# damaggu/StableKeypoints

Hardware: AMD Instinct MI355X
Metric: images/sec (token-opt step, 512², N=500 tokens) (higher is better)
Workload: dtype f32

## Files before the change

### stablekeypoints_amd/csrc/skp_conv.hip

```cpp
#include <cstdlib>

#include "skp_common.h"
#include "skp_gn.h"

using namespace skp;

#ifndef SKP_WINO_DEBUG
#define SKP_WINO_DEBUG 0
#endif
#ifndef SKP_WINO2_DEBUG
#define SKP_WINO2_DEBUG 0
#endif

namespace {

typedef float f32x4 __attribute__((ext_vector_type(4)));
typedef unsigned int u32x4 __attribute__((ext_vector_type(4)));

constexpr int kMT = 64;
constexpr int kNC = 32;
constexpr int kCK = 4;
constexpr int kP = 36;
constexpr int kThreads = 512;
constexpr int kUs = kCK * kNC * kP;
// ... 334 lines not shown
  SKP_CHECK_ARG(B > 0 && C > 0 && K > 0 && H > 0 && W > 0, "non-positive shape");
  SKP_CHECK_ARG(C % kCK == 0, "input channels must be a multiple of 4");
  SKP_CHECK_ARG(K % kNC == 0, "output channels must be a multiple of 32");
  SKP_CHECK_ARG(H % 4 == 0 && W % 4 == 0, "H and W must be multiples of 4");
  SKP_CHECK_ARG(nsplit >= 1 && C % (kCK * nsplit) == 0, "nsplit must divide C into multiples of 4");
  SKP_CHECK_ARG(nsplit == 1 || ws, "split-K needs a workspace of nsplit·B·K·H·W floats");
  SKP_CHECK_ARG(aligned16(x) && aligned16(U) && aligned16(y) && (!residual || aligned16(residual)) &&
                    (!ws || aligned16(ws)),
                "tensors must be 16-byte aligned");
  const int tw = W / 4, tpi = (H / 4) * tw;
  const long long ntiles = (long long)B * tpi;
  SKP_CHECK_ARG(ntiles <= 0x7fffffffLL - kMT, "too many tiles");
  SKP_CHECK_ARG((long long)B * C * H * W * 4 < 0x7fffffffLL, "input larger than 2 GiB (32-bit buffer offsets)");
  const bool wide = ntiles <= 32 && K % 64 == 0;
  const int mt = wide ? 32 : kMT;
  const int ntb = (int)((ntiles + mt - 1) / mt), nkb = K / (wide ? 64 : kNC);
  SKP_CHECK_ARG((long long)ntb * nkb * nsplit <= 0x7fffffffLL, "grid too large");
  const long long ubytes = (long long)K * C * kP * 4;
  const int kb_major = ubytes > (2LL << 20);
  const int epi = nsplit > 1 ? 0 : (bias ? 1 : 0) | (residual ? 2 : 0);
  float* out = nsplit > 1 ? ws : y;
  const int dbg = SKP_WINO_DEBUG;
  hipStream_t st = as_stream(stream);
  const dim3 grid((unsigned)(ntb * nkb * nsplit));
#define SKP_WG(E)                                                                                                    \
  if (wide)                                                                                                          \
    hipLaunchKernelGGL((wino_f4_kernel<E, 32>), grid, dim3(kThreads), 0, st, x, U, bias, residual, out, B, C, K, H, W, \
                       tw, tpi, (int)ntiles, ntb, nkb, kb_major, C / nsplit, dbg);                                    \
  else                                                                                                               \
    hipLaunchKernelGGL((wino_f4_kernel<E, 64>), grid, dim3(kThreads), 0, st, x, U, bias, residual, out, B, C, K, H, W, \
                       tw, tpi, (int)ntiles, ntb, nkb, kb_major, C / nsplit, dbg)
  switch (epi) {
    case 0: SKP_WG(0); break;
    case 1: SKP_WG(1); break;
    case 2: SKP_WG(2); break;
    default: SKP_WG(3); break;
  }
#undef SKP_WG
  SKP_LAUNCH_CHECK();
  if (nsplit > 1) return splitk_reduce(ws, nsplit, B, K, H * W, bias, residual, y, st);
  return SKP_OK;
}

namespace {
namespace w2 {

constexpr int kNC = 32;
constexpr int kCK = 4;
template <int TXB>
struct Geo;
template <>
struct Geo<8> {
  static constexpr int NI = 1, RR = 34, RC = 10, CHF = 1408;
};
template <>
struct Geo<4> {
  static constexpr int NI = 4, RR = 18, RC = 6, CHF = 1744;
};
template <int TXB, int NW>
struct GeoN : Geo<TXB> {};
template <>
struct GeoN<8, 4> {
  static constexpr int NI = 1, RR = 18, RC = 10, CHF = 768;
};
template <>
struct GeoN<4, 4> {
  static constexpr int NI = 2, RR = 18, RC = 6, CHF = 880;
};
template <int TXB, int NW = 8>
struct GeoT : GeoN<TXB, NW> {
  using GeoN<TXB, NW>::NI;
  using GeoN<TXB, NW>::RR;
  using GeoN<TXB, NW>::RC;
  using GeoN<TXB, NW>::CHF;
  static constexpr int RF = 4 * RC;
  static constexpr int RAWF = (4 * CHF + 255) / 256 * 256;
  static constexpr int RAW_INSTR = RAWF / 256;
  static_assert(NI * RR * RF <= CHF, "channel region");
};
constexpr int kUP = 40;
constexpr int kUF = kCK * kNC * kUP;
constexpr int kUInstr = kUF / 256;
constexpr unsigned kOOB = 0x80000000u;
static_assert(kUF % 256 == 0, "whole 1-KB chunks");
static_assert((4 * GeoT<8>::RAWF + 3 * kUF) * 4 <= 160 * 1024 && 3 * (GeoT<4>::RAWF + kUF) * 4 <= 160 * 1024, "LDS");
static_assert(2 * 8 * 1024 <= kUF * 4, "epilogue exchange: two waves' 8 KB per ring buffer");

__device__ constexpr float kBt[6][6] = {{1.f, -1.5f, -2.f, 1.5f, 1.f, 0.f},  {0.f, -1.f, 0.5f, 2.5f, 1.f, 0.f},
                                        {0.f, 1.f, -2.5f, 0.5f, 1.f, 0.f},  {0.f, -2.f, -1.f, 2.f, 1.f, 0.f},
                                        {0.f, 0.5f, -1.f, -0.5f, 1.f, 0.f}, {0.f, 1.f, -1.5f, -2.f, 1.5f, 1.f}};
__device__ constexpr float kAt[4][6] = {{1.f, 1.f, 1.f, 1.f, 1.f, 0.f},
                                        {0.f, 1.f, -1.f, 0.5f, -2.f, 0.f},
                                        {0.f, 1.f, 1.f, 0.25f, 4.f, 0.f},
                                        {0.f, 1.f, -1.f, 0.125f, -8.f, 1.f}};

#ifndef SKP_W2_PACKED
#define SKP_W2_PACKED 1
#endif
#if SKP_W2_PACKED
#define W2_TRANSFORM half_transform_pk
#else
#define W2_TRANSFORM half_transform
#endif

#define W2_VMCNT(n) __builtin_amdgcn_s_waitcnt(((n) & 15) | (((n) >> 4) << 14) | (7 << 4) | (15 << 8))

template <int H, int RF>
__device__ __forceinline__ void half_transform(const float* raw, float* a) {
  float t[3][6];
#pragma unroll
  for (int r = 0; r < 6; ++r) {
    const float4 c0 = *reinterpret_cast<const float4*>(raw + r * RF);
    const float4 c1 = *reinterpret_cast<const float4*>(raw + r * RF + 4);
    const float4 c2 = *reinterpret_cast<const float4*>(raw + r * RF + 8);
    const float d[6] = {c0.w, c1.x, c1.y, c1.z, c1.w, c2.x};
#pragma unroll
    for (int ii = 0; ii < 3; ++ii) {
      const float c = kBt[3 * H + ii][r];
      if (c == 0.0f) continue;
      bool first = true;
#pragma unroll
      for (int rp = 0; rp < r; ++rp)
        if (kBt[3 * H + ii][rp] != 0.0f) first = false;
#pragma unroll
      for (int b = 0; b < 6; ++b)
        t[ii][b] = first ? ((c == 1.0f) ? d[b] : c * d[b]) : ((c == 1.0f) ? t[ii][b] + d[b] : fmaf(c, d[b], t[ii][b]));
    }
    asm volatile("" ::"v"(c0.x), "v"(c0.y), "v"(c0.z), "v"(c2.y), "v"(c2.z), "v"(c2.w));
  }
#pragma unroll
  for (int ii = 0; ii < 3; ++ii) bt6(t[ii][0], t[ii][1], t[ii][2], t[ii][3], t[ii][4], t[ii][5], a + 6 * ii, 1);
}

typedef float f2 __attribute__((ext_vector_type(2)));

template <typename T>
__device__ __forceinline__ void bt6_shared(T a0, T a1, T a2, T a3, T a4, T a5, T* y) {
  const T e = a4 - a2, f = a3 - a1, g = a2 + a3, h = a3 - a2;
  y[0] = __builtin_elementwise_fma((T)1.5f, f, (a0 + e) - a2);
  y[1] = __builtin_elementwise_fma((T)1.5f, g, e + f);
  y[2] = __builtin_elementwise_fma((T)1.5f, h, e - f);
  y[3] = __builtin_elementwise_fma((T)2.0f, f, e);
  y[4] = __builtin_elementwise_fma((T)-0.5f, f, e);
  y[5] = __builtin_elementwise_fma((T)1.5f, e, __builtin_elementwise_fma((T)-2.0f, f, a5 - a1));
}

template <int H, int RF>
__device__ __forceinline__ void half_transform_pk(const float* raw, float* a) {
  f2 t[3][3];
  f2 k0[3], k1[3], k2[3], k3[3];
#pragma unroll
  for (int r = 0; r < 6; ++r) {
    if (H == 1 && r == 0) continue;
    const f32x4 c0 = *reinterpret_cast<const f32x4*>(raw + r * RF);
    const f32x4 c1 = *reinterpret_cast<const f32x4*>(raw + r * RF + 4);
    const f32x4 c2 = *reinterpret_cast<const f32x4*>(raw + r * RF + 8);
    const f2 d[3] = {__builtin_shufflevector(c1, c1, 0, 1), __builtin_shufflevector(c1, c1, 2, 3),
                     __builtin_shufflevector(c0, c2, 3, 4)};
#pragma unroll
    for (int p = 0; p < 3; ++p) {
      if (H == 0) {
        if (r == 0) k0[p] = d[p];
        if (r == 1) { k1[p] = d[p]; k0[p] = __builtin_elementwise_fma((f2)-1.5f, d[p], k0[p]); }
        if (r == 2) { k2[p] = d[p]; k3[p] = __builtin_elementwise_fma((f2)1.5f, d[p], -k1[p]); }
        if (r == 3) { k1[p] = __builtin_elementwise_fma((f2)1.5f, d[p], -k2[p]); k3[p] = k3[p] + d[p]; }
        if (r == 4) {
// ... 112 lines not shown

  unsigned voff[kMaxRaw];
  int nraw = 0;
#pragma unroll
  for (int m = 0; m < kMaxRaw; ++m) {
    const int gi = wv + NW * m;
    voff[m] = w2::kOOB;
    if (gi < kRawInstr) {
      ++nraw;
      const int f = 64 * gi + lane;
      const int ch = f / (kChF / 4);
      const int e = f - ch * (kChF / 4);
      const int ii = e / (RR * RC), rem = e - ii * (RR * RC);
      const int row = rem / RC, c4 = rem - row * RC;
      const int yy = y0 - 1 + row, xx = x0 - 4 + 4 * c4;
      if (ch < w2::kCK && ii < NI && yy >= 0 && yy < H && xx >= 0 && xx < W)
        voff[m] = (unsigned)((ximg + ((size_t)ii * C + ch) * plane + (size_t)yy * W + xx) * 4);
    }
  }
  const int nuw = (kInstr - 1 - wv) / NW + 1 - nraw;
  const int ufirst = wv + NW * nraw - kRawInstr;
  const int allow_step = RS == 2 ? 0 : US == 2 ? nraw : RS == 4 ? nuw + 2 * nraw : nuw + nraw;
  const int allow_pro = RS == 2 ? nuw + nraw : US == 2 ? nuw + 2 * nraw : RS == 4 ? 2 * nuw + 3 * nraw : 2 * nuw + 2 * nraw;
  const size_t xend = (size_t)(img + NI) * C * plane;
  const float* Ub = U + ((size_t)kb * C + c0) * w2::kNC * kUP;
  const int nst = csplit / w2::kCK;

  auto issue_raw = [&](int t, float* rs_lds) {
    const bool ok = t < nst;
    const size_t off = ((size_t)c0 + (size_t)(ok ? t : 0) * w2::kCK) * plane;
    const __amdgpu_buffer_rsrc_t rx = __builtin_amdgcn_make_buffer_rsrc(
        (void*)(x + off), (short)0, ok ? (int)((xend - off) * 4) : 0, 0x00020000);
#pragma unroll
    for (int m = 0; m < kMaxRaw; ++m)
      if (m < nraw && !(dbg & 4))
        __builtin_amdgcn_raw_ptr_buffer_load_lds(rx, (lds_ptr_t)(rs_lds + 256 * (wv + NW * m)), 16, voff[m], 0, 0, 0);
  };
  auto issue_u = [&](int t, float* us_lds) {
    const __amdgpu_buffer_rsrc_t ru =
        __builtin_amdgcn_make_buffer_rsrc((void*)(Ub + (size_t)t * kUF), (short)0, kUF * 4, 0x00020000);
#pragma unroll
    for (int m = 0; m < kMaxU; ++m)
      if (m < nuw && !(dbg & 8)) {
        const int q = ufirst + NW * m;
        __builtin_amdgcn_raw_ptr_buffer_load_lds(ru, (lds_ptr_t)(us_lds + 256 * q), 16, lane * 16, q * 1024, 0, 0);
      }
  };

  const int kc = lane >> 4;
  const int tx = lane & (TXB - 1);
  const int ty = TXB == 8 ? 2 * wm + ((lane >> 3) & 1) : (lane >> 2) & 3;
  const int roff = kc * kChF + (TXB == 8 ? 0 : wm * RR * kRowF) + 4 * ty * kRowF + 4 * tx;
  const int uoff = (kc * w2::kNC + (lane & 15)) * kUP + 20 * HH;

  f32x4 acc[2][18];
#pragma unroll
  for (int b = 0; b < 2; ++b)
#pragma unroll
    for (int q = 0; q < 18; ++q) acc[b][q] = f32x4{0.f, 0.f, 0.f, 0.f};
  float a0[18], a1[18];

  auto mfmas = [&](const float* us, const float (&acur)[18]) {
#pragma unroll
    for (int b = 0; b < 2; ++b) {
      const float* ub = us + uoff + b * 16 * kUP;
      float u[18];
#pragma unroll
      for (int j = 0; j < 4; ++j) {
        const float4 v = *reinterpret_cast<const float4*>(ub + 4 * j);
        u[4 * j] = v.x;
        u[4 * j + 1] = v.y;
        u[4 * j + 2] = v.z;
        u[4 * j + 3] = v.w;
      }
      const float2 v2 = *reinterpret_cast<const float2*>(ub + 16);
      u[16] = v2.x;
      u[17] = v2.y;
#pragma unroll
      for (int q = 0; q < 18; ++q) acc[b][q] = __builtin_amdgcn_mfma_f32_16x16x4f32(acur[q], u[q], acc[b][q], 0, 0, 0);
    }
  };

  if constexpr (VST) {
    const int bw = W >> 5;
    const size_t tb = (size_t)img * ((H >> 4) * bw) + (size_t)(y0 >> 4) * bw + (x0 >> 5);
    const float* Vb = x + (tb * (size_t)(C / w2::kCK) + (size_t)(c0 / w2::kCK)) * kUF;
    auto issue_vu = [&](int t, float* vs_lds, float* us_lds) {
      const __amdgpu_buffer_rsrc_t rv =
          __builtin_amdgcn_make_buffer_rsrc((void*)(Vb + (size_t)t * kUF), (short)0, kUF * 4, 0x00020000);
      const __amdgpu_buffer_rsrc_t ru =
          __builtin_amdgcn_make_buffer_rsrc((void*)(Ub + (size_t)t * kUF), (short)0, kUF * 4, 0x00020000);
#pragma unroll
      for (int m = 0; m < w2::kUInstr / NW; ++m) {
        const int q = wv + NW * m;
        __builtin_amdgcn_raw_ptr_buffer_load_lds(rv, (lds_ptr_t)(vs_lds + 256 * q), 16, lane * 16, q * 1024, 0, 0);
      }
#pragma unroll
      for (int m = 0; m < w2::kUInstr / NW; ++m) {
        const int q = wv + NW * m;
        __builtin_amdgcn_raw_ptr_buffer_load_lds(ru, (lds_ptr_t)(us_lds + 256 * q), 16, lane * 16, q * 1024, 0, 0);
      }
    };
    static_assert(w2::kUInstr % NW == 0, "whole chunks per wave");
    const int aoff = (kc * 32 + 16 * wm + (lane & 15)) * kUP + 20 * HH;
    auto vstep = [&](int s, const float* Vs, const float* Us, float* Vi, float* Ui) {
      W2_VMCNT(0);
      __syncthreads();
      if (s + 1 < nst) issue_vu(s + 1, Vi, Ui);
      float a[18];
      const float* vb = Vs + aoff;
#pragma unroll
      for (int j = 0; j < 4; ++j) {
        const float4 v = *reinterpret_cast<const float4*>(vb + 4 * j);
        a[4 * j] = v.x;
        a[4 * j + 1] = v.y;
        a[4 * j + 2] = v.z;
        a[4 * j + 3] = v.w;
      }
      const float2 v2 = *reinterpret_cast<const float2*>(vb + 16);
      a[16] = v2.x;
      a[17] = v2.y;
      mfmas(Us, a);
    };
    issue_vu(0, R0, U0);
    for (int s0 = 0; s0 < nst; s0 += 2) {
      vstep(s0, R0, U0, R1, U1);
      if (s0 + 1 < nst) vstep(s0 + 1, R1, U1, R0, U0);
    }
  } else {
    issue_raw(0, R0);
    if (RS == 4) issue_raw(1, R1);
    issue_u(0, U0);
    if (RS >= 3) issue_raw(RS - 2, RS == 4 ? R2 : R1);
    if (US == 3 && nst > 1) issue_u(1, U1);
    issue_raw(RS - 1, RS == 4 ? sm.R3 : RS == 3 ? R2 : R1);
    w2_vmcnt(nst > 1 ? allow_pro : 0);
    __syncthreads();
    w2::W2_TRANSFORM<HH, kRowF>(R0 + roff, a0);

    auto step = [&](int s, float* Rn, float* Us, float* Ri, float* Ui, const float (&acur)[18], float (&anext)[18]) {
      w2_vmcnt(s + 1 < nst ? allow_step : 0);
      __syncthreads();
      if (s + US - 1 < nst) issue_u(s + US - 1, Ui);
      issue_raw(s + RS, Ri);
      const bool tr = s + 1 < nst && !(dbg & 1);
      if (HH == 0) {
        if (tr) w2::W2_TRANSFORM<HH, kRowF>(Rn + roff, anext);
        if (!(dbg & 2)) mfmas(Us, acur);
      } else {
        if (!(dbg & 2)) mfmas(Us, acur);
        if (tr) w2::W2_TRANSFORM<HH, kRowF>(Rn + roff, anext);
      }
    };
    constexpr int PER = RS == 4 ? 12 : RS == 2 ? 2 : 6;
    float* const Rsl[4] = {R0, R1, R2, sm.R3};
    float* const Usl[3] = {U0, U1, U2};
    for (int s0 = 0; s0 < ((dbg & 16) ? 0 : nst); s0 += PER) {
      step(s0, Rsl[1 % RS], Usl[0], Rsl[0], Usl[US - 1], a0, a1);
  #pragma unroll
      for (int j = 1; j < PER; ++j) {
        if (s0 + j < nst) {
          if ((j & 1) == 0) step(s0 + j, Rsl[(j + 1) % RS], Usl[j % US], Rsl[j % RS], Usl[(j + US - 1) % US], a0, a1);
          else step(s0 + j, Rsl[(j + 1) % RS], Usl[j % US], Rsl[j % RS], Usl[(j + US - 1) % US], a1, a0);
        }
      }
    }

  }

  W2_VMCNT(0);
  __syncthreads();
  if (dbg & 32) return;
  constexpr int PH = (TXB == 8 && NW == 4) ? 16 : 32;
  constexpr int PLS = (TXB == 8 ? PH * 32 : NI * 256) + 4;
  float* const P2 = RS == 2 ? U1 : R2;
  auto plane_of = [&](int c) -> float* {
    float* b = (c >> 2) == 0 ? R0 : (c >> 2) == 1 ? R1 : (c >> 2) == 2 ? P2 : U0;
    return b + (c & 3) * PLS + (c >> 2) * 16;
  };
  float* pl = plane_of(lane & 15);
  const int pbase = TXB == 8 ? (4 * (2 * wm + (lane >> 5))) * 32 + 4 * (4 * ((lane >> 4) & 1))
                             : wm * 256 + (4 * (lane >> 4)) * 16;
  constexpr int PW = TXB == 8 ? 32 : 16;
#pragma unroll
  for (int blk = 0; blk < 2; ++blk) {
    if (HH != blk) {
#pragma unroll
      for (int r = 0; r < 4; ++r) {
        float m[18], o[16];
#pragma unroll
        for (int q = 0; q < 18; ++q) m[q] = acc[blk][q][r];
        w2::half_output<HH>(m, o);
#pragma unroll
        for (int f = 0; f < 4; ++f)
          *reinterpret_cast<float4*>(pl + pbase + f * PW + 4 * r) =
              make_float4(o[4 * f], o[4 * f + 1], o[4 * f + 2], o[4 * f + 3]);
      }
    }
    __syncthreads();
    if (HH == blk) {
#pragma unroll
      for (int r = 0; r < 4; ++r) {
        float m[18], o[16];
#pragma unroll
        for (int q = 0; q < 18; ++q) m[q] = acc[blk][q][r];
        w2::half_output<HH>(m, o);
#pragma unroll
        for (int f = 0; f < 4; ++f) {
          float4* d = reinterpret_cast<float4*>(pl + pbase + f * PW + 4 * r);
          const float4 p = *d;
// ... 90 lines not shown
        const float p = r == 0 ? piv[0] : r == 1 ? piv[1] : r == 2 ? piv[2] : piv[3];
        constexpr float inv_n = 1.0f / 512.0f;
        gnp[((size_t)img * K + k) * (size_t)((H >> 4) * (W >> 5)) + seg] =
            make_float2(p + x * inv_n, fmaxf(x2 - x * (x * inv_n), 0.0f));
      }
    }
    if (blk == 0) __syncthreads();
  }
}

template <int EPI, int TXB, int NW = 8>
__global__ __launch_bounds__(NW * WAVE) __attribute__((amdgpu_waves_per_eu(2, 2))) void wino2_kernel(
    const float* __restrict__ x, const float* __restrict__ U, const float* __restrict__ bias,
    const float* __restrict__ res, float* __restrict__ y, int nimg, int C, int K, int H, int W, int bw, int bpi,
    int nblk, int nkb, int kb_major, int csplit, int dbg, float2* __restrict__ gnp) {
  __shared__ __attribute__((aligned(16))) float R0[w2::GeoT<TXB, NW>::RAWF], R1[w2::GeoT<TXB, NW>::RAWF],
      R2[(TXB == 4 && NW == 4) ? 4 : w2::GeoT<TXB, NW>::RAWF],
      R3[(TXB == 8 && NW == 8 && SKP_W2_RS4) ? w2::GeoT<TXB, NW>::RAWF : 4];
  __shared__ __attribute__((aligned(16))) float U0[w2::kUF], U1[w2::kUF], U2[NW == 4 ? 4 : w2::kUF];
  const int G = gridDim.x;
  const int g = blockIdx.x;
  const int Lg = (G % 8 == 0) ? (g % 8) * (G / 8) + g / 8 : g;
  const int sp = Lg / (nblk * nkb);
  const int L = Lg - sp * (nblk * nkb);
  y += (size_t)sp * nimg * K * ((EPI & 4) ? (H / 2) * (W / 2) : H * W);
  int tb, kb;
  if (kb_major) {
    kb = L / nblk;
    tb = L - kb * nblk;
  } else {
    tb = L / nkb;
    kb = L - tb * nkb;
  }
  int img, x0 = 0, y0 = 0;
  if (TXB == 8) {
    img = tb / bpi;
    const int br = tb - img * bpi;
    const int by = br / bw;
    x0 = 32 * (br - by * bw);
    y0 = (NW == 4 ? 16 : 32) * by;
  } else {
    img = (NW == 4 ? 2 : 4) * tb;
  }
  const int wv = __builtin_amdgcn_readfirstlane(threadIdx.x >> 6);
  const W2Smem sm{R0, R1, R2, R3, U0, U1, U2};
  const int c0 = sp * csplit;
  if (wv < NW / 2)
    wino2_body<EPI, 0, TXB, NW>(sm, x, U, bias, res, y, C, K, H, W, img, x0, y0, kb, c0, csplit, wv, dbg, gnp);
  else wino2_body<EPI, 1, TXB, NW>(sm, x, U, bias, res, y, C, K, H, W, img, x0, y0, kb, c0, csplit, wv, dbg, gnp);
}

__global__ void wino2_weights_kernel(const float* __restrict__ w, int K, int C, int flip, float* __restrict__ U) {
  const long long i = blockIdx.x * (long long)blockDim.x + threadIdx.x;
  if (i >= (long long)K * C) return;
  const int k = (int)(i / C), c = (int)(i - (long long)k * C);
  double g[9];
  for (int u = 0; u < 3; ++u)
    for (int v = 0; v < 3; ++v)
      g[3 * u + v] = flip ? (double)w[((size_t)c * K + k) * 9 + (2 - u) * 3 + (2 - v)]
                          : (double)w[((size_t)k * C + c) * 9 + u * 3 + v];
  const double Gm[6][3] = {{1.0, 0.0, 0.0},
                           {1.0 / 3, 1.0 / 3, 1.0 / 3},
                           {-1.0 / 3, 1.0 / 3, -1.0 / 3},
                           {-16.0 / 15, -8.0 / 15, -4.0 / 15},
                           {1.0 / 15, -2.0 / 15, 4.0 / 15},
                           {0.0, 0.0, 1.0}};
  double t[6][3];
  for (int a = 0; a < 6; ++a)
    for (int v = 0; v < 3; ++v) t[a][v] = Gm[a][0] * g[v] + Gm[a][1] * g[3 + v] + Gm[a][2] * g[6 + v];
  float* out = U + (((size_t)(k / w2::kNC) * C + c) * w2::kNC + (k % w2::kNC)) * w2::kUP;
  for (int p = 0; p < w2::kUP; ++p) out[p] = 0.0f;
  for (int a = 0; a < 6; ++a)
    for (int b = 0; b < 6; ++b) {
      const int p = 6 * a + b;
      out[p < 18 ? p : p + 2] = (float)(t[a][0] * Gm[b][0] + t[a][1] * Gm[b][1] + t[a][2] * Gm[b][2]);
    }
}

template <int EPI>
__global__ __launch_bounds__(4 * WAVE) __attribute__((amdgpu_waves_per_eu(2, 2))) void wino2v_kernel(
    const float* __restrict__ V, const float* __restrict__ U, const float* __restrict__ bias,
    const float* __restrict__ res, float* __restrict__ y, int nimg, int C, int K, int H, int W, int bw, int bpi,
    int nblk, int nkb, int kb_major, int csplit, int dbg, float2* __restrict__ gnp) {
  __shared__ __attribute__((aligned(16))) float V0[w2::kUF], V1[w2::kUF], U0[w2::kUF], U1[w2::kUF];
  static_assert(4 * w2::kUF * 4 <= 80 * 1024, "two workgroups per CU");
  const int G = gridDim.x;
  const int g = blockIdx.x;
  const int Lg = (G % 8 == 0) ? (g % 8) * (G / 8) + g / 8 : g;
  const int sp = Lg / (nblk * nkb);
  const int L = Lg - sp * (nblk * nkb);
  y += (size_t)sp * nimg * K * H * W;
  int tb, kb;
  if (kb_major) {
    kb = L / nblk;
    tb = L - kb * nblk;
  } else {
    tb = L / nkb;
    kb = L - tb * nkb;
  }
  const int img = tb / bpi;
  const int br = tb - img * bpi;
  const int by = br / bw;
  const int x0 = 32 * (br - by * bw), y0 = 16 * by;
  const int wv = __builtin_amdgcn_readfirstlane(threadIdx.x >> 6);
  const W2Smem sm{V0, V1, nullptr, nullptr, U0, U1, nullptr};
  const int c0 = sp * csplit;
  if (wv < 2)
    wino2_body<EPI, 0, 8, 4, true>(sm, V, U, bias, res, y, C, K, H, W, img, x0, y0, kb, c0, csplit, wv, dbg, gnp);
  else wino2_body<EPI, 1, 8, 4, true>(sm, V, U, bias, res, y, C, K, H, W, img, x0, y0, kb, c0, csplit, wv, dbg, gnp);
}

template <int GN>
__global__ __launch_bounds__(4 * WAVE) void wino2_vtransform_kernel(
    const float* __restrict__ x, const float* __restrict__ stats, const float* __restrict__ gamma,
    const float* __restrict__ beta, const float* __restrict__ shift, int G, float* __restrict__ V, int C, int H, int W,
    int bw, int bpi) {
  using Geo = w2::GeoT<8, 4>;
  constexpr int RR = Geo::RR, RC = Geo::RC, kChF = Geo::CHF, kRowF = Geo::RF;
  __shared__ __attribute__((aligned(16))) float R[Geo::RAWF];
  __shared__ __attribute__((aligned(16))) float O[w2::kUF];
  const int tid = threadIdx.x, lane = tid & 63;
  const int nst = C / w2::kCK;
  const int tb = blockIdx.x / nst, st = blockIdx.x - tb * nst;
  const int img = tb / bpi;
  const int br = tb - img * bpi;
  const int by = br / bw;
  const int x0 = 32 * (br - by * bw), y0 = 16 * by;
  const int cpg = C / (G > 0 ? G : 1);
  for (int f = tid; f < w2::kCK * RR * RC; f += 4 * WAVE) {
    const int ch = f / (RR * RC), e = f - ch * (RR * RC);
    const int row = e / RC, c4 = e - row * RC;
    const int yy = y0 - 1 + row, xx = x0 - 4 + 4 * c4;
    float4 v = make_float4(0.f, 0.f, 0.f, 0.f);
    if (yy >= 0 && yy < H && xx >= 0 && xx < W) {
      const int c = w2::kCK * st + ch;
      v = *reinterpret_cast<const float4*>(x + (((size_t)img * C + c) * H + yy) * W + xx);
      if (GN) {
        const int grp = img * G + c / cpg;
        const GNCoef k = gn_coef(gamma[c], beta[c], stats[2 * grp], stats[2 * grp + 1]);
        const float t = shift ? shift[(size_t)img * C + c] : 0.0f;
        v.x = gn_elem<GN == 2>(v.x, t, k); v.y = gn_elem<GN == 2>(v.y, t, k);
        v.z = gn_elem<GN == 2>(v.z, t, k); v.w = gn_elem<GN == 2>(v.w, t, k);
      }
    }
    *reinterpret_cast<float4*>(R + ch * kChF + row * kRowF + 4 * c4) = v;
  }
  __syncthreads();
  const int wv = __builtin_amdgcn_readfirstlane(tid >> 6);
  const int HH = wv >> 1, wm = wv & 1;
  const int kc = lane >> 4, tx = lane & 7, ty = 2 * wm + ((lane >> 3) & 1);
  const int roff = kc * kChF + 4 * ty * kRowF + 4 * tx;
  float a[20];
  if (HH == 0) w2::W2_TRANSFORM<0, kRowF>(R + roff, a);
  else w2::W2_TRANSFORM<1, kRowF>(R + roff, a);
  a[18] = a[19] = 0.0f;
  float* o = O + (kc * 32 + 16 * wm + (lane & 15)) * w2::kUP + 20 * HH;
#pragma unroll
  for (int j = 0; j < 5; ++j)
    *reinterpret_cast<float4*>(o + 4 * j) = make_float4(a[4 * j], a[4 * j + 1], a[4 * j + 2], a[4 * j + 3]);
  __syncthreads();
  float4* out = reinterpret_cast<float4*>(V + (size_t)blockIdx.x * w2::kUF);
#pragma unroll
  for (int i = 0; i < w2::kUF / 4 / (4 * WAVE); ++i)
    out[i * 4 * WAVE + tid] = reinterpret_cast<const float4*>(O)[i * 4 * WAVE + tid];
}

}

extern "C" int skp_wino2_weights(const float* w, int K, int C, int flip, float* U, void* stream) {
  SKP_CHECK_ARG(w && U, "null pointer");
  SKP_CHECK_ARG(K > 0 && C > 0, "non-positive shape");
  SKP_CHECK_ARG(K % w2::kNC == 0, "output channels must be a multiple of 32");
  const long long n = (long long)K * C;
  hipLaunchKernelGGL(wino2_weights_kernel, dim3((unsigned)((n + 255) / 256)), dim3(256), 0, as_stream(stream), w, K, C,
                     flip, U);
  SKP_LAUNCH_CHECK();
  return SKP_OK;
}

namespace {
int wino_nt_flag(long long out_bytes, int nsplit) {
  if (nsplit > 1) return 0;
  return out_bytes >= (256LL << 20) ? 128 : 0;
}
}

extern "C" int skp_conv3x3s2_wino2(const float* x, const float* U, const float* bias, float* y, int B, int C, int K,
                                   int H, int W, int nsplit, float* ws, void* stream) {
  SKP_CHECK_ARG(x && U && y, "null pointer");
  SKP_CHECK_ARG(B > 0 && C > 0 && K > 0 && H > 0 && W > 0, "non-positive shape");
  SKP_CHECK_ARG(C % w2::kCK == 0, "input channels must be a multiple of 4");
  SKP_CHECK_ARG(K % w2::kNC == 0, "output channels must be a multiple of 32");
  SKP_CHECK_ARG(H % 32 == 0 && W % 32 == 0, "H and W must be multiples of 32");
  SKP_CHECK_ARG(nsplit >= 1 && C % (w2::kCK * nsplit) == 0, "nsplit must divide C into multiples of 4");
  SKP_CHECK_ARG(nsplit == 1 || ws, "split-K needs a workspace of nsplit·B·K·(H/2)·(W/2) floats");
  SKP_CHECK_ARG(aligned16(x) && aligned16(U) && aligned16(y) && (!ws || aligned16(ws)), "tensors must be 16-byte aligned");
  SKP_CHECK_ARG((long long)B * C * H * W * 4 < 0x7fffffffLL, "input larger than 2 GiB (32-bit buffer offsets)");
  const int bw = W / 32, bpi = (H / 16) * bw;
  const long long nblk = (long long)B * bpi;
  const int nkb = K / w2::kNC;
  SKP_CHECK_ARG(nblk * nkb * nsplit <= 0x7fffffffLL, "grid too large");
  float* out = nsplit > 1 ? ws : y;
  hipStream_t st = as_stream(stream);
  const dim3 grid((unsigned)(nblk * nkb * nsplit));
  const int fl = SKP_WINO2_DEBUG | wino_nt_flag((long long)B * K * (H / 2) * (W / 2) * 4, nsplit);
  if (nsplit == 1 && bias)
    hipLaunchKernelGGL((wino2_kernel<5, 8, 4>), grid, dim3(4 * WAVE), 0, st, x, U, bias, nullptr, out, B, C, K, H, W,
                       bw, bpi, (int)nblk, nkb, 0, C / nsplit, fl, nullptr);
  else
    hipLaunchKernelGGL((wino2_kernel<4, 8, 4>), grid, dim3(4 * WAVE), 0, st, x, U, nullptr, nullptr, out, B, C, K, H,
                       W, bw, bpi, (int)nblk, nkb, 0, C / nsplit, fl, nullptr);
  SKP_LAUNCH_CHECK();
  if (nsplit > 1) return splitk_reduce(ws, nsplit, B, K, (H / 2) * (W / 2), bias, nullptr, y, st);
  return SKP_OK;
}

extern "C" int skp_conv3x3_wino2_gn(const float* x, const float* U, const float* bias, const float* residual, float* y,
                                    int B, int C, int K, int H, int W, int nsplit, float* ws, float* gn_part,
                                    void* stream) {
  SKP_CHECK_ARG(x && U && y, "null pointer");
  SKP_CHECK_ARG(!gn_part || (nsplit == 1 && H % 32 == 0 && W % 32 == 0 && (reinterpret_cast<uintptr_t>(gn_part) & 7) == 0),
                "gn_part: one split, H and W multiples of 32, 8-byte aligned");
  SKP_CHECK_ARG(B > 0 && C > 0 && K > 0 && H > 0 && W > 0, "non-positive shape");
  SKP_CHECK_ARG(C % w2::kCK == 0, "input channels must be a multiple of 4");
  SKP_CHECK_ARG(K % w2::kNC == 0, "output channels must be a multiple of 32");
  const bool g16 = H == 16 && W == 16;
  SKP_CHECK_ARG((H % 32 == 0 && W % 32 == 0) || (g16 && B % 4 == 0),
                "H and W must be multiples of 32, or 16×16 with B a multiple of 4");
  SKP_CHECK_ARG(nsplit >= 1 && C % (w2::kCK * nsplit) == 0, "nsplit must divide C into multiples of 4");
  SKP_CHECK_ARG(nsplit == 1 || ws, "split-K needs a workspace of nsplit·B·K·H·W floats");
  SKP_CHECK_ARG(aligned16(x) && aligned16(U) && aligned16(y) && (!residual || aligned16(residual)) &&
                    (!ws || aligned16(ws)),
                "tensors must be 16-byte aligned");
  SKP_CHECK_ARG((long long)B * C * H * W * 4 < 0x7fffffffLL, "input larger than 2 GiB (32-bit buffer offsets)");
  const int bw = W / 32, bpi = (H / 16) * bw;
  const long long nblk = g16 ? B / 2 : (long long)B * bpi;
  const int nkb = K / w2::kNC;
  SKP_CHECK_ARG(nblk * nkb * nsplit <= 0x7fffffffLL, "grid too large");
  const int dbg = SKP_WINO2_DEBUG;
  const int kb_major = 0;
  const int epi = nsplit > 1 ? 0 : (bias ? 1 : 0) | (residual ? 2 : 0);
  float* out = nsplit > 1 ? ws : y;
  hipStream_t st = as_stream(stream);
  const dim3 grid((unsigned)(nblk * nkb * nsplit));
  const int fl = dbg | wino_nt_flag((long long)B * K * H * W * 4, nsplit);
  float2* gnp = reinterpret_cast<float2*>(gn_part);
#define SKP_WG2(E)                                                                                            \
// ... 110 lines not shown
```

### stablekeypoints_amd/ops.py

```python
import ctypes
import os

import torch

from . import _lib
from ._lib import call, ptr, stream

F32 = torch.float32

_TIMER = None


def set_kernel_timer(timer):
    global _TIMER
    _TIMER = timer


class _NoTimer:
    def __enter__(self):
        return self

    def __exit__(self, *a):
        return False

# ... 1550 lines not shown
def conv3x3_s2(x, weight, bias=None):
    _lib.require_device(x)
    if not conv3x3_s2_eligible(x, weight):
        raise ValueError(f"conv3x3_s2: unsupported x {tuple(x.shape)} / weight {tuple(weight.shape)}")
    x = _c16(x)
    B, C, H, W = x.shape
    K = weight.shape[0]
    y = torch.empty(B, K, H // 2, W // 2, device=x.device, dtype=F32)
    U = _wino_u(weight, False, True)
    b = None if bias is None else _c(bias.detach())
    bmax = max(1, (2 ** 31 - 1) // (C * H * W * 4))
    for b0 in range(0, B, bmax):
        b1 = min(B, b0 + bmax)
        _, nsplit, _ = _wino_plan(b1 - b0, C, K, H, W)
        ws = torch.empty(nsplit, b1 - b0, K, H // 2, W // 2, device=x.device, dtype=F32) if nsplit > 1 else None
        with _timed("skp_conv3x3s2_wino2", 0):
            call("skp_conv3x3s2_wino2", ptr(x[b0:b1]), ptr(U), ptr(b), ptr(y[b0:b1]), b1 - b0, C, K, H, W, nsplit,
                 ptr(ws), stream(x.device))
    return y


def conv3x3(x, weight, bias=None, residual=None):
    _lib.require_device(x)
    if weight.requires_grad:
        raise ValueError("conv3x3: the weight must be frozen (requires_grad=False)")
    B, C, H, W = x.shape
    K = weight.shape[0]
    if tuple(weight.shape[1:]) != (C, 3, 3):
        raise ValueError(f"conv3x3: weight {tuple(weight.shape)} does not fit input {tuple(x.shape)}")
    if residual is not None and tuple(residual.shape) != (B, K, H, W):
        raise ValueError(f"conv3x3: residual {tuple(residual.shape)} is not ({B}, {K}, {H}, {W})")
    if C % 4 and C < 16 and x.dtype == F32 and wino_eligible(B, C + 4 - C % 4, K, H, W):
        pad = 4 - C % 4
        xp = torch.nn.functional.pad(x, (0, 0, 0, 0, 0, pad))
        wp = torch.nn.functional.pad(weight.detach(), (0, 0, 0, 0, 0, pad))
        return Conv3x3.apply(xp, wp, bias, residual)
    if x.dtype != F32 or not wino_eligible(B, C, K, H, W):
        y = torch.nn.functional.conv2d(x, weight, bias, 1, 1)
        return y if residual is None else residual + y
    return Conv3x3.apply(x, weight, bias, residual)


WINO_V_SHAPES = {(512, 512, 64, 64), (256, 512, 128, 128), (512, 512, 128, 128), (128, 256, 256, 256),
                 (256, 256, 256, 256)}
WINO_V_MIN_BATCH = 4


def gn_conv3x3_wins(B, C, K, H, W):
    return ((C, K, H, W) in WINO_V_SHAPES and B >= WINO_V_MIN_BATCH and C % 4 == 0 and K % 32 == 0
            and H % 32 == 0 and W % 32 == 0 and WINO_KERNEL == "auto" and not _wino_gemm_ok(B, C, K, H, W))


def gn_conv3x3(x, gamma, beta, groups, eps, act, shift, weight, bias=None, residual=None):
    _lib.require_device(x)
    if torch.is_grad_enabled() and (x.requires_grad or (residual is not None and residual.requires_grad)):
        raise ValueError("gn_conv3x3: forward only (no gradient reaches the normalised activation)")
    if weight.requires_grad or gamma.requires_grad or beta.requires_grad:
        raise ValueError("gn_conv3x3: the parameters must be frozen")
    pre = _gn_parts_of(x) if GN_EPI else None
    x = _c16(x.detach())
    B, C, H, W = x.shape
    K = weight.shape[0]
    if tuple(weight.shape[1:]) != (C, 3, 3):
        raise ValueError(f"gn_conv3x3: weight {tuple(weight.shape)} does not fit input {tuple(x.shape)}")
    if residual is not None:
        if tuple(residual.shape) != (B, K, H, W):
            raise ValueError(f"gn_conv3x3: residual {tuple(residual.shape)} is not ({B}, {K}, {H}, {W})")
        residual = _c16(residual.detach())
    if shift is not None:
        shift = _c(shift.detach().reshape(-1, C).to(x.device, F32).expand(B, C))
    dev = x.device
    nws = _lib.lib().skp_groupnorm_workspace(B, C, H * W, int(groups))
    if nws < 0:
        raise ValueError(f"gn_conv3x3: bad shape {tuple(x.shape)} groups={groups}")
    part = torch.empty(nws, device=dev, dtype=torch.float64)
    stats = torch.empty(B * groups * 2, device=dev, dtype=F32)
    g, b = _c(gamma.detach()), _c(beta.detach())
    if pre is not None:
        call("skp_groupnorm_stats_part", ptr(pre[0]), pre[1], ptr(shift), B, C, H * W, int(groups), float(eps),
             ptr(stats), ptr(part), stream(dev))
    else:
        call("skp_groupnorm_stats", ptr(x), ptr(shift), B, C, H * W, int(groups), float(eps), ptr(stats), ptr(part),
             stream(dev))
    V = torch.empty(B * C * (H // 4) * (W // 4) * 40, device=dev, dtype=F32)
    with _timed("skp_wino2_vtransform_gn", 0):
        call("skp_wino2_vtransform_gn", ptr(x), ptr(stats), ptr(g), ptr(b), ptr(shift), int(groups), int(bool(act)),
             ptr(V), B, C, H, W, stream(dev))
    _, nsplit, _ = _wino_plan(B, C, K, H, W)
    U = _wino_u(weight, False, True)
    y = torch.empty(B, K, H, W, device=dev, dtype=F32)
    ws = torch.empty(nsplit, B, K, H, W, device=dev, dtype=F32) if nsplit > 1 else None
    gnp = torch.empty(B, K, (H // 16) * (W // 32), 2, device=dev, dtype=F32) if GN_EPI and nsplit == 1 else None
    bias = None if bias is None else _c(bias.detach())
    with _timed("skp_conv3x3_wino2_v", 0):
        call("skp_conv3x3_wino2_v_gn", ptr(V), ptr(U), ptr(bias), ptr(residual), ptr(y), B, C, K, H, W, nsplit,
             ptr(ws), ptr(gnp), stream(dev))
    if gnp is not None:
        y._skp_gn = (y._version, gnp, gnp.shape[2])
    return y


TAB10 = ((31, 119, 180), (255, 127, 14), (44, 160, 44), (214, 39, 40), (148, 103, 189), (140, 86, 75),
         (227, 119, 194), (127, 127, 127), (188, 189, 34), (23, 190, 207))
_VIRIDIS_ANCHORS = ((0, (0.267004, 0.004874, 0.329415)), (32, (0.278826, 0.175490, 0.483397)),
                    (64, (0.229739, 0.322361, 0.545706)), (96, (0.172719, 0.448791, 0.557885)),
                    (128, (0.127568, 0.566949, 0.550556)), (160, (0.157851, 0.683765, 0.501686)),
                    (192, (0.369214, 0.788888, 0.382914)), (224, (0.678489, 0.863742, 0.189503)),
                    (255, (0.993248, 0.906157, 0.143936)))
_LUT_CACHE = {}


def default_colors(K):
    if K <= 10:
        rows = TAB10[:K]
    else:
        import colorsys
        rows = [tuple(int(round(255 * c)) for c in colorsys.hsv_to_rgb(j / K, 0.9, 1.0)) for j in range(K)]
    return torch.tensor(rows, dtype=torch.uint8).reshape(K, 3)


def fallback_lut():
    lut = torch.empty(256, 3, dtype=F32)
    for (i0, c0), (i1, c1) in zip(_VIRIDIS_ANCHORS[:-1], _VIRIDIS_ANCHORS[1:]):
        t = torch.arange(i0, i1 + 1, dtype=torch.float64).sub(i0).div(i1 - i0)[:, None]
        lut[i0:i1 + 1] = (torch.tensor(c0, dtype=torch.float64) * (1 - t) + torch.tensor(c1, dtype=torch.float64) * t).float()
    return lut.clamp_(0.0, 1.0)


def default_lut():
    try:
        import matplotlib
        import numpy as np
        cm = matplotlib.colormaps["viridis"]
        return torch.tensor(np.asarray(cm(np.linspace(0.0, 1.0, 256)))[:, :3], dtype=F32).contiguous()
    except ImportError:
        return fallback_lut()


def map_range(maps):
    _lib.require_device(maps)
    maps = _c(maps)
    n, h, w = maps.shape
    out = torch.empty(n, 2, device=maps.device, dtype=F32)
    call("skp_map_range", ptr(maps), n, h, w, ptr(out), stream(maps.device))
    return out


def sheet_shape(H, W, rows, cols, downscale=1, pad=2):
    return rows * (H // downscale + pad) + pad, cols * (W // downscale + pad) + pad


def render_sheet(images, maps=None, points=None, *, rows, cols, downscale=1, pad=2, alpha=0.7, radius=None,
                 colors=None, lut=None, overlay=None):
    _lib.require_device(images, maps, points)
    images = _c(images)
    n, C, H, W = images.shape
    if C != 3:
        raise ValueError(f"render_sheet: images must be (n, 3, H, W), got {tuple(images.shape)}")
    dev = images.device
    f = int(downscale)
    h = w = 0
    rng = None
    if maps is not None:
        maps = _c(maps)
        if maps.dim() != 3 or maps.shape[0] != n:
            raise ValueError(f"render_sheet: maps must be ({n}, h, w), got {tuple(maps.shape)}")
        h, w = maps.shape[1:]
# ... 66 lines not shown
```

Measured before the change: 44.20.

## Store Winograd V in per-wave register layout and load it directly into VGPRs

The pre-transformed Winograd input V is now written in a per-wave, lane-contiguous layout with no padding (36 floats per tile instead of 40). The V-stationary conv loop loads it straight into registers with buffer loads instead of staging it through LDS. It also moves to a three-deep U ring buffer with prefetch two stages ahead. The transform kernel drops its LDS staging and barrier. Together these cut V traffic and LDS use, in exchange for more VGPR pressure and hand-tuned waitcnt and barrier sequencing that could be fragile.

```diff
diff --git a/stablekeypoints_amd/csrc/skp_conv.hip b/stablekeypoints_amd/csrc/skp_conv.hip
--- a/stablekeypoints_amd/csrc/skp_conv.hip
+++ b/stablekeypoints_amd/csrc/skp_conv.hip
@@ -440,6 +440,9 @@
 constexpr int kUF = kCK * kNC * kUP;
 constexpr int kUInstr = kUF / 256;
 constexpr unsigned kOOB = 0x80000000u;
+constexpr int kVWF = 4 * 256 + 128;
+constexpr int kVF = 4 * kVWF;
+typedef unsigned int u32x2 __attribute__((ext_vector_type(2)));
 static_assert(kUF % 256 == 0, "whole 1-KB chunks");
 static_assert((4 * GeoT<8>::RAWF + 3 * kUF) * 4 <= 160 * 1024 && 3 * (GeoT<4>::RAWF + kUF) * 4 <= 160 * 1024, "LDS");
 static_assert(2 * 8 * 1024 <= kUF * 4, "epilogue exchange: two waves' 8 KB per ring buffer");
@@ -718,19 +721,26 @@
   };
 
   if constexpr (VST) {
+    using w2::kVF;
+    using w2::kVWF;
     const int bw = W >> 5;
     const size_t tb = (size_t)img * ((H >> 4) * bw) + (size_t)(y0 >> 4) * bw + (x0 >> 5);
-    const float* Vb = x + (tb * (size_t)(C / w2::kCK) + (size_t)(c0 / w2::kCK)) * kUF;
-    auto issue_vu = [&](int t, float* vs_lds, float* us_lds) {
+    const float* Vb = x + (tb * (size_t)(C / w2::kCK) + (size_t)(c0 / w2::kCK)) * kVF + wv * kVWF;
+    asm volatile("" : "+s"(Vb));
+    struct AReg {
+      u32x4 c[4];
+      w2::u32x2 d;
+    };
+    auto issue_vu = [&](int t, AReg& an, float* us_lds) {
+      const bool ok = t < nst;
+      const size_t tt = ok ? (size_t)t : 0;
       const __amdgpu_buffer_rsrc_t rv =
-          __builtin_amdgcn_make_buffer_rsrc((void*)(Vb + (size_t)t * kUF), (short)0, kUF * 4, 0x00020000);
+          __builtin_amdgcn_make_buffer_rsrc((void*)(Vb + tt * kVF), (short)0, ok ? kVWF * 4 : 0, 0x00020000);
       const __amdgpu_buffer_rsrc_t ru =
-          __builtin_amdgcn_make_buffer_rsrc((void*)(Ub + (size_t)t * kUF), (short)0, kUF * 4, 0x00020000);
-#pragma unroll
-      for (int m = 0; m < w2::kUInstr / NW; ++m) {
-        const int q = wv + NW * m;
-        __builtin_amdgcn_raw_ptr_buffer_load_lds(rv, (lds_ptr_t)(vs_lds + 256 * q), 16, lane * 16, q * 1024, 0, 0);
-      }
+          __builtin_amdgcn_make_buffer_rsrc((void*)(Ub + tt * kUF), (short)0, ok ? kUF * 4 : 0, 0x00020000);
+#pragma unroll
+      for (int j = 0; j < 4; ++j) an.c[j] = __builtin_amdgcn_raw_buffer_load_b128(rv, lane * 16, j * 1024, 0);
+      an.d = __builtin_amdgcn_raw_buffer_load_b64(rv, lane * 8, 4096, 0);
 #pragma unroll
       for (int m = 0; m < w2::kUInstr / NW; ++m) {
         const int q = wv + NW * m;
@@ -738,30 +748,40 @@
       }
     };
     static_assert(w2::kUInstr % NW == 0, "whole chunks per wave");
-    const int aoff = (kc * 32 + 16 * wm + (lane & 15)) * kUP + 20 * HH;
-    auto vstep = [&](int s, const float* Vs, const float* Us, float* Vi, float* Ui) {
-      W2_VMCNT(0);
-      __syncthreads();
-      if (s + 1 < nst) issue_vu(s + 1, Vi, Ui);
-      float a[18];
-      const float* vb = Vs + aoff;
-#pragma unroll
-      for (int j = 0; j < 4; ++j) {
-        const float4 v = *reinterpret_cast<const float4*>(vb + 4 * j);
-        a[4 * j] = v.x;
-        a[4 * j + 1] = v.y;
-        a[4 * j + 2] = v.z;
-        a[4 * j + 3] = v.w;
-      }
-      const float2 v2 = *reinterpret_cast<const float2*>(vb + 16);
-      a[16] = v2.x;
-      a[17] = v2.y;
-      mfmas(Us, a);
+    constexpr int kPerStage = 5 + w2::kUInstr / NW;
+    auto vstep = [&](int s, const AReg& ac, const float* Us, AReg& ai, float* Ui) {
+      W2_VMCNT(kPerStage);
+      asm volatile("" ::: "memory");
+      __builtin_amdgcn_s_waitcnt(0xC07F);
+      __builtin_amdgcn_s_barrier();
+      asm volatile("" ::: "memory");
+      asm volatile("" ::"v"(ac.c[0]), "v"(ac.c[1]), "v"(ac.c[2]), "v"(ac.c[3]), "v"(ac.d));
+      issue_vu(s + 2, ai, Ui);
+      __builtin_amdgcn_sched_barrier(0);
+      if (s < nst) {
+        float a[18];
+#pragma unroll
+        for (int j = 0; j < 4; ++j)
+#pragma unroll
+          for (int i = 0; i < 4; ++i) {
+            const unsigned v = ac.c[j][i];
+            a[4 * j + i] = __uint_as_float(v);
+          }
+        const unsigned d0 = ac.d[0], d1 = ac.d[1];
+        a[16] = __uint_as_float(d0);
+        a[17] = __uint_as_float(d1);
+        mfmas(Us, a);
+      }
     };
-    issue_vu(0, R0, U0);
-    for (int s0 = 0; s0 < nst; s0 += 2) {
-      vstep(s0, R0, U0, R1, U1);
-      if (s0 + 1 < nst) vstep(s0 + 1, R1, U1, R0, U0);
+    AReg A0, A1, A2;
+    issue_vu(0, A0, U0);
+    asm volatile("" ::: "memory");
+    __builtin_amdgcn_sched_barrier(0);
+    issue_vu(1, A1, U1);
+    for (int s0 = 0; s0 < nst; s0 += 3) {
+      vstep(s0, A0, U0, A2, U2);
+      vstep(s0 + 1, A1, U1, A0, U0);
+      vstep(s0 + 2, A2, U2, A1, U1);
     }
   } else {
     issue_raw(0, R0);
@@ -1018,8 +1038,9 @@
     const float* __restrict__ V, const float* __restrict__ U, const float* __restrict__ bias,
     const float* __restrict__ res, float* __restrict__ y, int nimg, int C, int K, int H, int W, int bw, int bpi,
     int nblk, int nkb, int kb_major, int csplit, int dbg, float2* __restrict__ gnp) {
-  __shared__ __attribute__((aligned(16))) float V0[w2::kUF], V1[w2::kUF], U0[w2::kUF], U1[w2::kUF];
-  static_assert(4 * w2::kUF * 4 <= 80 * 1024, "two workgroups per CU");
+  __shared__ __attribute__((aligned(16))) float U0[w2::kUF], U1[w2::kUF], U2[w2::kUF];
+  static_assert(3 * w2::kUF * 4 <= 80 * 1024, "two workgroups per CU");
+  static_assert(4 * (16 * 32 + 4) + 48 <= w2::kUF / 2, "a plane buffer per half U slot");
   const int G = gridDim.x;
   const int g = blockIdx.x;
   const int Lg = (G % 8 == 0) ? (g % 8) * (G / 8) + g / 8 : g;
@@ -1039,7 +1060,7 @@
   const int by = br / bw;
   const int x0 = 32 * (br - by * bw), y0 = 16 * by;
   const int wv = __builtin_amdgcn_readfirstlane(threadIdx.x >> 6);
-  const W2Smem sm{V0, V1, nullptr, nullptr, U0, U1, nullptr};
+  const W2Smem sm{U0 + w2::kUF / 2, U1 + w2::kUF / 2, nullptr, nullptr, U0, U1, U2};
   const int c0 = sp * csplit;
   if (wv < 2)
     wino2_body<EPI, 0, 8, 4, true>(sm, V, U, bias, res, y, C, K, H, W, img, x0, y0, kb, c0, csplit, wv, dbg, gnp);
@@ -1054,7 +1075,6 @@
   using Geo = w2::GeoT<8, 4>;
   constexpr int RR = Geo::RR, RC = Geo::RC, kChF = Geo::CHF, kRowF = Geo::RF;
   __shared__ __attribute__((aligned(16))) float R[Geo::RAWF];
-  __shared__ __attribute__((aligned(16))) float O[w2::kUF];
   const int tid = threadIdx.x, lane = tid & 63;
   const int nst = C / w2::kCK;
   const int tb = blockIdx.x / nst, st = blockIdx.x - tb * nst;
@@ -1086,19 +1106,14 @@
   const int HH = wv >> 1, wm = wv & 1;
   const int kc = lane >> 4, tx = lane & 7, ty = 2 * wm + ((lane >> 3) & 1);
   const int roff = kc * kChF + 4 * ty * kRowF + 4 * tx;
-  float a[20];
+  float a[18];
   if (HH == 0) w2::W2_TRANSFORM<0, kRowF>(R + roff, a);
   else w2::W2_TRANSFORM<1, kRowF>(R + roff, a);
-  a[18] = a[19] = 0.0f;
-  float* o = O + (kc * 32 + 16 * wm + (lane & 15)) * w2::kUP + 20 * HH;
-#pragma unroll
-  for (int j = 0; j < 5; ++j)
-    *reinterpret_cast<float4*>(o + 4 * j) = make_float4(a[4 * j], a[4 * j + 1], a[4 * j + 2], a[4 * j + 3]);
-  __syncthreads();
-  float4* out = reinterpret_cast<float4*>(V + (size_t)blockIdx.x * w2::kUF);
-#pragma unroll
-  for (int i = 0; i < w2::kUF / 4 / (4 * WAVE); ++i)
-    out[i * 4 * WAVE + tid] = reinterpret_cast<const float4*>(O)[i * 4 * WAVE + tid];
+  float* o = V + (size_t)blockIdx.x * w2::kVF + wv * w2::kVWF;
+#pragma unroll
+  for (int j = 0; j < 4; ++j)
+    *reinterpret_cast<float4*>(o + 256 * j + 4 * lane) = make_float4(a[4 * j], a[4 * j + 1], a[4 * j + 2], a[4 * j + 3]);
+  *reinterpret_cast<float2*>(o + 1024 + 2 * lane) = make_float2(a[16], a[17]);
 }
 
 }
diff --git a/stablekeypoints_amd/ops.py b/stablekeypoints_amd/ops.py
--- a/stablekeypoints_amd/ops.py
+++ b/stablekeypoints_amd/ops.py
@@ -1656,7 +1656,7 @@
     else:
         call("skp_groupnorm_stats", ptr(x), ptr(shift), B, C, H * W, int(groups), float(eps), ptr(stats), ptr(part),
              stream(dev))
-    V = torch.empty(B * C * (H // 4) * (W // 4) * 40, device=dev, dtype=F32)
+    V = torch.empty(B * C * (H // 4) * (W // 4) * 36, device=dev, dtype=F32)
     with _timed("skp_wino2_vtransform_gn", 0):
         call("skp_wino2_vtransform_gn", ptr(x), ptr(stats), ptr(g), ptr(b), ptr(shift), int(groups), int(bool(act)),
              ptr(V), B, C, H, W, stream(dev))
```

Result: faster. 44.72, median of 6 (+1.2%).
